# retab-dev/k-LLMs

Hardware: NVIDIA H100
Metric: consensus records/sec at n=16 (1M x 32-field); achieved HBM GB/s vs peak (higher is better)
Workload: dtype i32 codes / f64 values

## Files before the change

### k_llms_b200/csrc/kc_jsongpu.cu

```cuda
#include <cuda_runtime.h>

#include <algorithm>
#include <atomic>
#include <chrono>
#include <cstdio>
#include <cstdlib>
#include <cstring>
#include <mutex>
#include <string>
#include <thread>
#include <type_traits>
#include <vector>

#include <cub/device/device_scan.cuh>
#include <nvtx3/nvToolsExt.h>

#include "../../include/kllms_b200.h"
#include "kc_internal.h"
#include "kc_jsongpu.cuh"

namespace {

using kc::js::Chunk;
using kc::js::Tok;

#define R_(call)                              \
    do {                                      \
        if (const int rc_ = (call)) return rc_; \
    } while (0)

struct DBuf {
    void *p = nullptr;
    size_t cap = 0;
    int reserve(size_t need) {
        if (p && need <= cap) return KC_OK;
        if (p) cudaFree(p);
        p = nullptr;
        cap = 0;
        need += need / 8 + 256;
        if (cudaMalloc(&p, need) != cudaSuccess) {
            cudaGetLastError();
            return kc_fail(KC_ENOMEM, "kc_consolidate_json_packed: cudaMalloc(%zu) failed", need);
        }
        cap = need;
        return KC_OK;
    }
    int grow(size_t need, size_t keep, cudaStream_t s) {
        if (!keep) return reserve(need);
        if (p && need <= cap) return KC_OK;
        void *old = p;
        const size_t old_cap = cap;
        p = nullptr;
        cap = 0;
        if (const int rc = reserve(need)) {
            cudaFree(old);
            return rc;
        }
        if (old) KC_CUDA_I(cudaMemcpyAsync(p, old, std::min(keep, old_cap), cudaMemcpyDeviceToDevice, s));
        KC_CUDA_I(cudaStreamSynchronize(s));
        if (old) cudaFree(old);
        return KC_OK;
    }
    template <typename T>
    T *as() const { return static_cast<T *>(p); }
};

struct PBuf {
    void *p = nullptr;
    size_t cap = 0;
    int reserve(size_t need) {
        if (p && need <= cap) return KC_OK;
        if (p) cudaFreeHost(p);
        p = nullptr;
        cap = 0;
        need += need / 8 + 256;
        if (cudaHostAlloc(&p, need, cudaHostAllocDefault) != cudaSuccess) {
            cudaGetLastError();
            return kc_fail(KC_ENOMEM, "kc_consolidate_json_packed: cudaHostAlloc(%zu) failed", need);
        }
        cap = need;
        return KC_OK;
    }
    template <typename T>
    T *as() const { return static_cast<T *>(p); }
};

enum Stage { RECORDS, SLOTS, UNION, SCRATCH, CSR, OFF };
struct Units {
    size_t R, B, T = 0, P = 0, S = 0;
};
template <class Alloc>
int chunk_arrays(const Alloc &alloc, Chunk &ch, Stage stage, const Units &u, size_t keep, bool vrec) {
    const size_t n = (size_t)ch.n;
    int k = 0;
    auto a = [&](Stage st, auto *&ptr, size_t count, size_t per, size_t plus, int fill, bool on_device) {
        const int i = k++;
        return st == stage ? alloc(i, ptr, count * per + plus, keep * per, fill, on_device) : KC_OK;
    };
    R_(a(RECORDS, ch.fcount, u.R, 1, 1, 0, true));
    R_(a(RECORDS, ch.slot, u.R, 1, 1, 0, false));
    R_(a(RECORDS, ch.status, u.R, 1, 0, 0, false));
    R_(a(RECORDS, ch.nest, u.R, 1, 0, 0, false));
    R_(a(RECORDS, ch.pend, u.R, 1, 0, 0, false));
    R_(a(RECORDS, ch.plist, u.R, 1, 1, 0xFF, false));
    R_(a(ch.lists ? RECORDS : OFF, ch.lst, u.R, 1, 0, 0, false));
    R_(a(RECORDS, ch.vbase, u.R, 1, 0, 0, false));
    R_(a(RECORDS, ch.xbase, u.R, 1, 0, 0, false));
    R_(a(RECORDS, ch.mcount, u.R, 1, 1, 0, true));
    R_(a(RECORDS, ch.scount, u.R, 1, 1, 0, true));
    R_(a(RECORDS, ch.ccount, u.R, 1, 1, 0, true));
    R_(a(RECORDS, ch.len_c, u.R, 1, 1, 0, true));
    R_(a(RECORDS, ch.len_l, u.R, 1, 1, 0, true));
    R_(a(SLOTS, ch.toks, u.T, n, 1, 0, false));
    R_(a(SLOTS, ch.fdesc, u.T, 1, 1, 0, false));
    R_(a(SLOTS, ch.gpos, u.T, 1, 1, 0, false));
    R_(a(SLOTS, ch.piece_c, u.T, 1, 1, 0, false));
    R_(a(SLOTS, ch.piece_l, u.T, 1, 1, 0, false));
    R_(a(SLOTS, ch.vcells, u.T, n, 16, 0xFF, true));
    R_(a(SLOTS, ch.xcells, u.T, n, 2, 0, true));
    R_(a(vrec ? SLOTS : OFF, ch.vrec, u.T, 1, 1, 0xFF, false));
    R_(a(UNION, ch.ucand, u.P, n, 0, 0, false));
    R_(a(UNION, ch.ubase, u.P, 1, 0, 0, false));
    R_(a(UNION, ch.usize, u.P, 1, 0, 0, false));
    R_(a(SCRATCH, ch.utok, u.S, 1, 0, 0, false));
    R_(a(SCRATCH, ch.unode, u.S, 1, 0, 0, false));
    R_(a(SCRATCH, ch.umap, u.S, 1, 0, 0xFF, false));
    R_(a(CSR, ch.mchars, u.B, 1, 16, 0, false));
    R_(a(CSR, ch.mstr_off, u.T, n, 2, 0, false));
    R_(a(CSR, ch.mgrp_off, u.T, 1, 2, 0, false));
    return KC_OK;
}

void set_flags(Chunk &ch, uint32_t flags, uint8_t lists, int32_t aligned0) {
    ch.xmedoid = (flags & KC_JSON_NUMERIC_MEDOID) != 0;
    ch.key_union = (flags & KC_JSON_KEY_UNION) != 0;
    ch.unicode = (flags & KC_JSON_UNICODE) != 0;
    ch.lists = lists;
    ch.aligned0 = aligned0;
}

struct Worker {
    int device = -1;
    cudaStream_t stream = nullptr;
    cudaEvent_t ev[7] = {};
    DBuf text, off, counters, win, vmeta, xvalue, xmeta, out_c, out_l, scan_tmp, midx, mavg, seq, vweight;
    std::vector<DBuf> arrays;
    PBuf h_small;
    PBuf h_scan;
    bool busy = false;
    int init(int dev) {
        if (device == dev) return KC_OK;
        KC_CUDA_I(cudaStreamCreateWithFlags(&stream, cudaStreamNonBlocking));
        for (auto &e : ev) KC_CUDA_I(cudaEventCreate(&e));
        device = dev;
        return KC_OK;
    }
};

std::mutex g_pool_mu;
std::vector<Worker *> g_workers;

Worker *acquire_worker(int device) {
    std::lock_guard<std::mutex> lock(g_pool_mu);
    for (Worker *w : g_workers)
        if (!w->busy && w->device == device) {
            w->busy = true;
            return w;
        }
    Worker *w = new Worker;
    w->busy = true;
    g_workers.push_back(w);
    return w;
}
void release_worker(Worker *w) {
    std::lock_guard<std::mutex> lock(g_pool_mu);
    w->busy = false;
}

struct PinnedBlob {
    char *p = nullptr;
    size_t cap = 0;
};
std::vector<PinnedBlob> g_blob_pool;

PinnedBlob acquire_blob(size_t need) {
    {
        std::lock_guard<std::mutex> lock(g_pool_mu);
        int best = -1;
        for (int i = 0; i < (int)g_blob_pool.size(); ++i)
            if (g_blob_pool[i].cap >= need && (best < 0 || g_blob_pool[i].cap < g_blob_pool[best].cap)) best = i;
        if (best >= 0) {
            PinnedBlob b = g_blob_pool[best];
            g_blob_pool.erase(g_blob_pool.begin() + best);
            return b;
        }
    }
    PinnedBlob b;
    void *p = nullptr;
    if (cudaHostAlloc(&p, need, cudaHostAllocDefault) != cudaSuccess) {
        cudaGetLastError();
        return b;
    }
    b.p = (char *)p;
    b.cap = need;
    return b;
}
void release_blob(PinnedBlob b) {
    if (!b.p) return;
    std::lock_guard<std::mutex> lock(g_pool_mu);
    size_t n_small = 0, n_large = 0;
    for (auto &x : g_blob_pool) (x.cap <= ((size_t)4 << 20) ? n_small : n_large)++;
    if (b.cap <= ((size_t)4 << 20) && n_small < 64) {
        g_blob_pool.push_back(b);
        return;
    }
    if (n_large >= 4 || b.cap <= ((size_t)4 << 20)) {
        int smallest = -1;
        for (int i = 0; i < (int)g_blob_pool.size(); ++i)
            if (g_blob_pool[i].cap > ((size_t)4 << 20) && (smallest < 0 || g_blob_pool[i].cap < g_blob_pool[smallest].cap)) smallest = i;
        if (smallest < 0 || g_blob_pool[smallest].cap >= b.cap) {
            cudaFreeHost(b.p);
            return;
        }
        cudaFreeHost(g_blob_pool[smallest].p);
        g_blob_pool.erase(g_blob_pool.begin() + smallest);
    }
    g_blob_pool.push_back(b);
}

int team_size(int n) {
    int t = 2;
    while (t < n && t < 32) t *= 2;
    return t;
}

int device_arrays(Worker &w, Chunk &ch, Stage stage, const Units &u, size_t keep, bool weighted) {
    auto dev = [&](int k, auto *&ptr, size_t len, size_t keep_len, int fill, bool on_device) -> int {
        using E = std::remove_reference_t<decltype(*ptr)>;
        if (w.arrays.size() <= (size_t)k) w.arrays.resize((size_t)k + 1);
        R_(w.arrays[(size_t)k].grow(len * sizeof(E), keep_len * sizeof(E), w.stream));
        ptr = w.arrays[(size_t)k].as<E>();
        if (on_device) KC_CUDA_I(cudaMemsetAsync(ptr + keep_len, fill, (len - keep_len) * sizeof(E), w.stream));
        return KC_OK;
    };
    R_(chunk_arrays(dev, ch, stage, u, keep, weighted));
    if (stage != SLOTS) return KC_OK;
    const size_t T1 = std::max<size_t>(u.T, 1);
    R_(w.win.reserve(T1 * 4));
    R_(w.vmeta.reserve(T1 * 4));
    R_(w.xvalue.reserve(T1 * 8));
    R_(w.xmeta.reserve(T1 * 4));
    ch.vmeta = w.vmeta.as<uint32_t>();
    ch.xvalue = w.xvalue.as<double>();
    ch.xmeta = w.xmeta.as<uint32_t>();
    ch.xbest = w.xmeta.as<int32_t>();
    ch.xavg = w.xvalue.as<double>();
    if (weighted) {
        R_(w.vweight.reserve(T1 * 4));
        ch.vweight = w.vweight.as<float>();
    }
    return KC_OK;
}

template <typename T>
void exclusive_scan(T *v, size_t len) {
    T acc = 0;
    for (size_t i = 0; i < len; ++i) {
        const T c = v[i];
        v[i] = acc;
        acc += c;
    }
}

}

struct kc_json_result {
    int64_t R = 0;
    PinnedBlob blob;
    std::atomic<int64_t> used{0};
    std::vector<int64_t> c_off, c_len, l_off, l_len;
    std::vector<uint8_t> status, why;
    std::string heap;
    kc_json_stats stats{};
};

namespace {

struct ChunkStage {
    float h2d = 0, plan = 0, kernels = 0, emit = 0, d2h = 0;
};

int union_round(Worker &w, Chunk &ch, Units &u, int team, int grid, bool weighted, unsigned long long *h_cnt) {
    cudaStream_t s = w.stream;
    const int32_t P = (int32_t)u.P;
    R_(device_arrays(w, ch, UNION, u, 0, weighted));
    ch.uslot = (uint32_t)u.T;
    kc::js::union_count_kernel<<<grid, 128, 0, s>>>(ch, team, P);
    KC_CUDA_I(cudaGetLastError());
    KC_CUDA_I(cudaMemcpyAsync(h_cnt, ch.counters, 48, cudaMemcpyDeviceToHost, s));
    KC_CUDA_I(cudaStreamSynchronize(s));
    u.S = std::max<size_t>(h_cnt[4], 1);
    if (u.S >= ((size_t)1 << 32)) return kc_fail(KC_EINVAL, "kc_consolidate_json_packed: %zu union scratch entries in one chunk", u.S);
    R_(device_arrays(w, ch, SCRATCH, u, 0, weighted));
    kc::js::union_build_kernel<<<grid, 128, 0, s>>>(ch, team, P);
    KC_CUDA_I(cudaGetLastError());
    KC_CUDA_I(cudaMemcpyAsync(h_cnt, ch.counters, 48, cudaMemcpyDeviceToHost, s));
    KC_CUDA_I(cudaStreamSynchronize(s));
    if (const size_t U = h_cnt[5]) {
        const size_t keep = u.T;
        u.T += U;
        if (u.T >= ((size_t)1 << 32)) return kc_fail(KC_EINVAL, "kc_consolidate_json_packed: %zu field slots in one chunk", u.T);
        R_(device_arrays(w, ch, SLOTS, u, keep, weighted));
    }
    kc::js::union_plan_kernel<<<grid, 128, 0, s>>>(ch, team, P);
    KC_CUDA_I(cudaGetLastError());
    KC_CUDA_I(cudaMemcpyAsync(h_cnt, ch.counters, 48, cudaMemcpyDeviceToHost, s));
    KC_CUDA_I(cudaStreamSynchronize(s));
    return KC_OK;
}

int run_chunk(Worker &w, const char *h_text, const int64_t *h_off, const float *h_seq, uint32_t flags, uint8_t lists, const int64_t *dst,
              int64_t r0, int64_t r1, int32_t n, double rel_eps, double abs_eps, int sm_count, kc_json_result &res, ChunkStage &st) {
    const int64_t Rc = r1 - r0;
    const int64_t b0 = h_off[r0 * n], b1 = h_off[r1 * n];
    const size_t bytes = (size_t)(b1 - b0);
    if (bytes >= ((size_t)1 << 32)) return kc_fail(KC_EINVAL, "kc_consolidate_json_packed: chunk of %zu bytes", bytes);
    cudaStream_t s = w.stream;
    const bool weighted = h_seq != nullptr;
    Chunk ch{};
    ch.R = (int32_t)Rc;
    ch.n = n;
    set_flags(ch, flags, lists, INT32_MAX);
    Units u{(size_t)Rc, bytes};
    R_(device_arrays(w, ch, RECORDS, u, 0, weighted));
    R_(w.text.reserve(bytes + 16));
    R_(w.off.reserve((size_t)(Rc * n + 1) * 8));
    R_(w.counters.reserve(48));
    R_(w.h_small.reserve(64));
    R_(w.h_scan.reserve((size_t)(Rc + 1) * 16 + (size_t)Rc));
    if (h_seq) R_(w.seq.reserve((size_t)std::max<int64_t>(Rc * n, 1) * 4));
    size_t tmp_bytes = 0, tmp_bytes32 = 0;
    cub::DeviceScan::ExclusiveSum(nullptr, tmp_bytes, (const int64_t *)nullptr, (int64_t *)nullptr, (int)(Rc + 1), s);
    cub::DeviceScan::ExclusiveSum(nullptr, tmp_bytes32, (const uint32_t *)nullptr, (uint32_t *)nullptr, (int)(Rc + 1), s);
    R_(w.scan_tmp.reserve(std::max(tmp_bytes, tmp_bytes32) + 256));
    ch.text = w.text.as<uint8_t>();
    ch.off = w.off.as<int64_t>();
    ch.counters = w.counters.as<unsigned long long>();

    nvtxRangePushA("kc_json: H2D texts");
    KC_CUDA_I(cudaEventRecord(w.ev[0], s));
    KC_CUDA_I(cudaMemcpyAsync(w.text.p, h_text + b0, bytes, cudaMemcpyHostToDevice, s));
    KC_CUDA_I(cudaMemcpyAsync(w.off.p, h_off + r0 * n, (size_t)(Rc * n + 1) * 8, cudaMemcpyHostToDevice, s));
    if (h_seq) KC_CUDA_I(cudaMemcpyAsync(w.seq.p, h_seq + r0 * n, (size_t)(Rc * n) * 4, cudaMemcpyHostToDevice, s));
    KC_CUDA_I(cudaEventRecord(w.ev[1], s));
    nvtxRangePop();
    nvtxRangePushA("kc_json: plan (A0 count, A1 scan/type/encode)");

    const int team = team_size(n);
    const int tpw = 32 / team;
    auto grid_for = [&](int64_t threads_needed) {
        const int64_t blocks = (threads_needed + 127) / 128;
        return (int)std::max<int64_t>(1, std::min<int64_t>(blocks, (int64_t)sm_count * 16));
    };
    auto team_grid = [&](int64_t units) { return grid_for((units + tpw - 1) / tpw * 32); };
    kc::js::count_kernel<<<grid_for(Rc), 128, 0, s>>>(ch);
    KC_CUDA_I(cudaGetLastError());
    size_t tb = w.scan_tmp.cap;
    KC_CUDA_I(cub::DeviceScan::ExclusiveSum(w.scan_tmp.p, tb, (const uint32_t *)ch.fcount, ch.slot, (int)(Rc + 1), s));
    uint32_t *h_total = w.h_small.as<uint32_t>();
    KC_CUDA_I(cudaMemcpyAsync(h_total, ch.slot + Rc, 4, cudaMemcpyDeviceToHost, s));
    KC_CUDA_I(cudaStreamSynchronize(s));
    u.T = *h_total;
    R_(device_arrays(w, ch, SLOTS, u, 0, weighted));
    KC_CUDA_I(cudaMemsetAsync(w.counters.p, 0, 48, s));
    int64_t gv = 0, gx = 0, gm = 0;
    if (u.T) {
        kc::js::plan_kernel<<<team_grid(Rc), 128, 0, s>>>(ch, team);
        KC_CUDA_I(cudaGetLastError());
        unsigned long long *h_cnt = w.h_small.as<unsigned long long>() + 1;
        KC_CUDA_I(cudaMemcpyAsync(h_cnt, w.counters.p, 32, cudaMemcpyDeviceToHost, s));
        KC_CUDA_I(cudaStreamSynchronize(s));
        if ((u.P = h_cnt[3]))
            R_(union_round(w, ch, u, team, team_grid((int64_t)u.P), weighted, h_cnt));
        gv = (int64_t)h_cnt[0];
        gx = (int64_t)h_cnt[1];
        gm = (int64_t)h_cnt[2];
    }
    if (gm) {
        R_(device_arrays(w, ch, CSR, u, 0, weighted));
        R_(w.midx.reserve((u.T + 1) * 4));
        R_(w.mavg.reserve((u.T + 1) * 8));
        ch.midx = w.midx.as<int32_t>();
        ch.mavg = w.mavg.as<double>();
        for (uint32_t *cnt : {ch.mcount, ch.scount, ch.ccount}) {
            tb = w.scan_tmp.cap;
            KC_CUDA_I(cub::DeviceScan::ExclusiveSum(w.scan_tmp.p, tb, (const uint32_t *)cnt, cnt, (int)(Rc + 1), s));
        }
        kc::js::medoid_kernel<<<team_grid(Rc), 128, 0, s>>>(ch, team);
        KC_CUDA_I(cudaGetLastError());
    }
    KC_CUDA_I(cudaEventRecord(w.ev[2], s));
    nvtxRangePop();
    nvtxRangePushA("kc_json: K1 vote + K2 numeric + K4 medoid");
    if (gv && h_seq)
        R_(kc_weighted_vote_groups_i8(ch.vcells, gv, n, ch.vrec, w.seq.as<float>(), Rc, w.win.as<int32_t>(), w.vmeta.as<uint32_t>(),
                                      w.vweight.as<float>(), s));
    else if (gv)
        R_(kc_vote_i8(ch.vcells, gv, n, nullptr, 1, w.win.as<int32_t>(), w.vmeta.as<uint32_t>(), s));
    if (gx && ch.xmedoid) R_(kc_numeric_medoid_f64(ch.xcells, gx, n, w.xmeta.as<int32_t>(), w.xvalue.as<double>(), s));
    else if (gx) R_(kc_numeric_f64(ch.xcells, gx, n, rel_eps, abs_eps, w.xvalue.as<double>(), w.xmeta.as<uint32_t>(), s));
    if (gm) R_(kc_medoid_str(ch.mchars, ch.mstr_off, ch.mgrp_off, gm, std::max(2, n), w.midx.as<int32_t>(), w.mavg.as<double>(), s));
    KC_CUDA_I(cudaEventRecord(w.ev[3], s));
    nvtxRangePop();
    nvtxRangePushA("kc_json: emit (C0 lengths, C1 write)");
    kc::js::len_kernel<<<team_grid(Rc), 128, 0, s>>>(ch, team);
    KC_CUDA_I(cudaGetLastError());
    tb = w.scan_tmp.cap;
    KC_CUDA_I(cub::DeviceScan::ExclusiveSum(w.scan_tmp.p, tb, (const int64_t *)ch.len_c, ch.len_c, (int)(Rc + 1), s));
    tb = w.scan_tmp.cap;
    KC_CUDA_I(cub::DeviceScan::ExclusiveSum(w.scan_tmp.p, tb, (const int64_t *)ch.len_l, ch.len_l, (int)(Rc + 1), s));
    int64_t *h_scan_c = w.h_scan.as<int64_t>(), *h_scan_l = h_scan_c + (Rc + 1);
    uint8_t *h_status = (uint8_t *)(h_scan_l + (Rc + 1));
    KC_CUDA_I(cudaMemcpyAsync(h_scan_c, ch.len_c, (size_t)(Rc + 1) * 8, cudaMemcpyDeviceToHost, s));
    KC_CUDA_I(cudaMemcpyAsync(h_scan_l, ch.len_l, (size_t)(Rc + 1) * 8, cudaMemcpyDeviceToHost, s));
    KC_CUDA_I(cudaMemcpyAsync(h_status, ch.status, (size_t)Rc, cudaMemcpyDeviceToHost, s));
    KC_CUDA_I(cudaStreamSynchronize(s));
    const int64_t out_c_bytes = h_scan_c[Rc], out_l_bytes = h_scan_l[Rc];
    R_(w.out_c.reserve((size_t)std::max<int64_t>(out_c_bytes, 1)));
    R_(w.out_l.reserve((size_t)std::max<int64_t>(out_l_bytes, 1)));
    ch.out_c = w.out_c.as<uint8_t>();
    ch.out_l = w.out_l.as<uint8_t>();
    if (out_c_bytes) {
        kc::js::write_kernel<<<team_grid(Rc), 128, 0, s>>>(ch, team);
        KC_CUDA_I(cudaGetLastError());
    }
    KC_CUDA_I(cudaEventRecord(w.ev[4], s));
    nvtxRangePop();
    nvtxRangePushA("kc_json: D2H texts");
    const int64_t need = out_c_bytes + out_l_bytes;
    const int64_t pos = res.used.fetch_add(need);
    if (pos + need > (int64_t)res.blob.cap) {
        res.used.fetch_sub(need);
        for (int64_t i = r0; i < r1; ++i) {
            const int64_t r = dst ? dst[i] : i;
            res.status[(size_t)r] = 1;
            res.why[(size_t)r] = (uint8_t)kc::js::D_TOO_LONG;
        }
        return KC_OK;
    }
    if (out_c_bytes) KC_CUDA_I(cudaMemcpyAsync(res.blob.p + pos, ch.out_c, (size_t)out_c_bytes, cudaMemcpyDeviceToHost, s));
    if (out_l_bytes) KC_CUDA_I(cudaMemcpyAsync(res.blob.p + pos + out_c_bytes, ch.out_l, (size_t)out_l_bytes, cudaMemcpyDeviceToHost, s));
    KC_CUDA_I(cudaEventRecord(w.ev[5], s));
    KC_CUDA_I(cudaStreamSynchronize(s));
    nvtxRangePop();
    for (int64_t i = 0; i < Rc; ++i) {
        const int64_t r = dst ? dst[r0 + i] : r0 + i;
        res.status[(size_t)r] = h_status[i] ? 1 : 0;
        res.why[(size_t)r] = h_status[i];
        res.c_off[(size_t)r] = pos + h_scan_c[i];
        res.c_len[(size_t)r] = h_scan_c[i + 1] - h_scan_c[i];
        res.l_off[(size_t)r] = pos + out_c_bytes + h_scan_l[i];
        res.l_len[(size_t)r] = h_scan_l[i + 1] - h_scan_l[i];
    }
    float ms = 0;
    cudaEventElapsedTime(&ms, w.ev[0], w.ev[1]); st.h2d += ms;
    cudaEventElapsedTime(&ms, w.ev[1], w.ev[2]); st.plan += ms;
    cudaEventElapsedTime(&ms, w.ev[2], w.ev[3]); st.kernels += ms;
    cudaEventElapsedTime(&ms, w.ev[3], w.ev[4]); st.emit += ms;
    cudaEventElapsedTime(&ms, w.ev[4], w.ev[5]); st.d2h += ms;
    return KC_OK;
}

}

namespace {

void gather(const char *h_text, const int64_t *h_off, int32_t n, const std::vector<int64_t> &idx, std::vector<const char *> &texts,
            std::vector<int64_t> &lens) {
    texts.resize(idx.size() * n);
    lens.resize(idx.size() * n);
    for (size_t i = 0; i < idx.size(); ++i)
        for (int32_t c = 0; c < n; ++c) {
            const int64_t k = idx[i] * n + c;
            texts[i * n + c] = h_text + h_off[k];
            lens[i * n + c] = h_off[k + 1] - h_off[k];
        }
}

template <class Alloc>
int align_listed(const char *h_text, const int64_t *h_off, int32_t n, int device, int32_t threads, const std::vector<int64_t> &idx, const Alloc &alloc,
                 char *&blob, std::vector<int64_t> &off, std::vector<int64_t> &dst, std::vector<int64_t> &declined) {
    const int64_t L = (int64_t)idx.size();
    std::vector<const char *> texts;
    std::vector<int64_t> lens;
    gather(h_text, h_off, n, idx, texts, lens);
    std::vector<char *> out((size_t)(L * n), nullptr);
    std::vector<int32_t> st((size_t)L, 0);
    if (const int rc = kc_align_json_batch(texts.data(), lens.data(), L, n, 0.51, device, threads, out.data(), st.data(), nullptr)) {
        kc_free_strings(out.data(), L * n);
        return rc;
    }
    off.assign(1, 0);
    dst.clear();
    declined.clear();
    for (int64_t i = 0; i < L; ++i) {
        if (st[(size_t)i] != 0) {
            declined.push_back(idx[(size_t)i]);
            continue;
        }
        dst.push_back(idx[(size_t)i]);
        for (int32_t c = 0; c < n; ++c) off.push_back(off.back() + (int64_t)strlen(out[(size_t)(i * n + c)]));
    }
    blob = alloc((size_t)off.back());
    int rc = blob ? KC_OK : kc_fail(KC_ENOMEM, "kc_consolidate_json_packed: cannot allocate %lld bytes of aligned texts", (long long)off.back());
    for (int64_t i = 0, k = 0; i < L && !rc; ++i) {
        if (st[(size_t)i] != 0) continue;
        for (int32_t c = 0; c < n; ++c, ++k) memcpy(blob + off[(size_t)k], out[(size_t)(i * n + c)], (size_t)(off[(size_t)k + 1] - off[(size_t)k]));
    }
    kc_free_strings(out.data(), L * n);
    return rc;
}

template <class Round>
int list_round(kc_json_result &res, const char *h_text, const int64_t *h_off, const float *h_seq, int32_t n, int device, int32_t threads,
               Round &run_round) {
    std::vector<int64_t> idx;
    for (int64_t r = 0; r < res.R; ++r)
        if (res.status[(size_t)r] && res.why[(size_t)r] == kc::js::D_LIST) idx.push_back(r);
    if (idx.empty()) return KC_OK;
    PinnedBlob texts;
    auto alloc = [&](size_t bytes) {
        texts = acquire_blob(bytes + 16);
        return texts.p;
    };
    char *blob = nullptr;
    std::vector<int64_t> off, dst, declined;
    const int sim_device = idx.size() >= 64 ? device : -1;
    int rc = align_listed(h_text, h_off, n, sim_device, threads, idx, alloc, blob, off, dst, declined);
    for (int64_t r : declined) res.why[(size_t)r] = kc::js::D_ALIGN;
    const int64_t M = (int64_t)dst.size();
    if (!rc && M) {
        std::vector<float> seq;
        if (h_seq) {
            seq.resize((size_t)(M * n));
            for (int64_t i = 0; i < M; ++i) memcpy(&seq[(size_t)(i * n)], h_seq + dst[(size_t)i] * n, (size_t)n * 4);
        }
        size_t est = 4096;
        for (int64_t i = 0; i < M; ++i) {
            const char *t = blob + off[(size_t)(i * n)];
            const int64_t len = off[(size_t)(i * n + 1)] - off[(size_t)(i * n)];
            int64_t tokens = 1;
            for (int64_t k = 0; k < len; ++k) tokens += t[k] == ',' ? 1 : (t[k] == ']' || t[k] == '}') ? 2 : 0;
            est += (size_t)(2 * len + 32 * tokens);
        }
        const size_t need = (size_t)res.used.load() + est;
        if (need > res.blob.cap) {
            PinnedBlob bigger = acquire_blob(need);
            if (!bigger.p) rc = kc_fail(KC_ENOMEM, "kc_consolidate_json_packed: cannot grow the pinned output blob to %zu bytes", need);
            else {
                memcpy(bigger.p, res.blob.p, (size_t)res.used.load());
                release_blob(res.blob);
                res.blob = bigger;
            }
        }
        if (!rc) rc = run_round(blob, off.data(), h_seq ? seq.data() : nullptr, M, (uint8_t)2, dst.data());
    }
    release_blob(texts);
    return rc;
}

}

extern "C" {

namespace {

int consolidate_packed(const char *h_text, const int64_t *h_off, const float *h_seq, int64_t n_records, int32_t n, double rel_eps,
                       double abs_eps, int device, int32_t threads, uint32_t flags, kc_json_result **out) {
    if (!out) return kc_fail(KC_EINVAL, "kc_consolidate_json_packed: NULL out");
    if (h_seq || (flags & KC_JSON_NUMERIC_MEDOID)) flags |= KC_JSON_DEVICE_ONLY;
    *out = nullptr;
    if (n < 2 || n > KC_MAX_CANDIDATES) return kc_fail(KC_EINVAL, "kc_consolidate_json_packed: n=%d outside [2,%d]", n, KC_MAX_CANDIDATES);
    if (n_records < 0 || (n_records && (!h_text || !h_off))) return kc_fail(KC_EINVAL, "kc_consolidate_json_packed: bad arguments");
    if (!(rel_eps >= 0.0) || !(abs_eps >= 0.0)) return kc_fail(KC_EINVAL, "kc_consolidate_json_packed: rel_eps/abs_eps must be >= 0");
    const auto t_start = std::chrono::steady_clock::now();
    int prev = 0;
    KC_CUDA_I(cudaGetDevice(&prev));
    KC_CUDA_I(cudaSetDevice(device));
    int sm_count = 0, cc_major = 0;
    KC_CUDA_I(cudaDeviceGetAttribute(&sm_count, cudaDevAttrMultiProcessorCount, device));
    KC_CUDA_I(cudaDeviceGetAttribute(&cc_major, cudaDevAttrComputeCapabilityMajor, device));
    if (cc_major != 9) {
        cudaSetDevice(prev);
        return kc_fail(KC_ENODEV, "device %d has compute capability %d.x; this library is sm_90a only", device, cc_major);
    }
    kc_json_result *res = new (std::nothrow) kc_json_result;
    if (!res) return kc_fail(KC_ENOMEM, "kc_consolidate_json_packed: out of memory");
    const int64_t R = n_records;
    res->R = R;
    res->c_off.assign((size_t)R, 0);
    res->c_len.assign((size_t)R, 0);
    res->l_off.assign((size_t)R, 0);
    res->l_len.assign((size_t)R, 0);
    res->status.assign((size_t)R, 1);
    res->why.assign((size_t)R, 0);
    const int64_t total_bytes = R ? h_off[R * n] - h_off[0] : 0;
    res->blob = acquire_blob((size_t)(total_bytes / n * 3 + (1 << 20)));
    if (!res->blob.p) {
        delete res;
        cudaSetDevice(prev);
        return kc_fail(KC_ENOMEM, "kc_consolidate_json_packed: cannot allocate the pinned output blob");
    }
    size_t chunk_bytes = (size_t)64 << 20;
    if (const char *e = getenv("KC_JSON_CHUNK_MB")) chunk_bytes = (size_t)std::min(1024, std::max(1, atoi(e))) << 20;
    int max_workers = 3;
    if (const char *e = getenv("KC_JSON_STREAMS")) max_workers = std::max(1, std::min(8, atoi(e)));
    int n_chunks = 0, n_streams = 0;
    std::vector<ChunkStage> stages((size_t)max_workers);
    auto run_round = [&](const char *text, const int64_t *off, const float *seq, int64_t Rb, uint8_t lists, const int64_t *dst) -> int {
        std::vector<int64_t> cuts{0};
        int64_t r = 0;
        while (r < Rb) {
            const int64_t start = off[r * n];
            int64_t lo = r + 1, hi = Rb;
            while (lo < hi) {
                const int64_t mid = lo + (hi - lo + 1) / 2;
                if ((size_t)(off[mid * n] - start) <= chunk_bytes) lo = mid;
                else hi = mid - 1;
            }
            r = lo;
            cuts.push_back(r);
        }
        const int chunks = (int)cuts.size() - 1;
        const int n_workers = std::max(1, std::min(max_workers, chunks));
        n_chunks += chunks;
        n_streams = std::max(n_streams, n_workers);
        std::vector<Worker *> workers;
        for (int i = 0; i < n_workers; ++i) workers.push_back(acquire_worker(device));
        std::vector<int> rcs((size_t)n_workers, KC_OK);
        std::vector<std::string> errs((size_t)n_workers);
        std::atomic<int> next{0};
        auto body = [&](int wi) {
            cudaSetDevice(device);
            Worker &w = *workers[(size_t)wi];
            int rc = w.init(device);
            while (!rc) {
                const int k = next.fetch_add(1);
                if (k >= chunks) break;
                rc = run_chunk(w, text, off, seq, flags, lists, dst, cuts[(size_t)k], cuts[(size_t)k + 1], n, rel_eps, abs_eps, sm_count, *res,
                               stages[(size_t)wi]);
            }
            if (rc) {
                cudaStreamSynchronize(w.stream);
                errs[(size_t)wi] = kc_last_error();
            }
            rcs[(size_t)wi] = rc;
        };
        if (n_workers == 1) {
            body(0);
        } else {
            std::vector<std::thread> pool;
            for (int i = 0; i < n_workers; ++i) pool.emplace_back(body, i);
            for (auto &t : pool) t.join();
        }
        for (Worker *w : workers) release_worker(w);
        for (int i = 0; i < n_workers; ++i)
            if (rcs[(size_t)i]) return kc_fail(rcs[(size_t)i], "%s", errs[(size_t)i].c_str());
        return KC_OK;
    };
    const bool lists = (flags & KC_JSON_LISTS) != 0;
    int rc = run_round(h_text, h_off, h_seq, R, lists ? 1 : 0, nullptr);
    if (!rc && lists) rc = list_round(*res, h_text, h_off, h_seq, n, device, threads, run_round);
    const auto t_gpu = std::chrono::steady_clock::now();
    int64_t n_declined = 0, n_host = 0;
    if (!rc) {
        std::vector<int64_t> idx;
        for (int64_t r = 0; r < R; ++r) {
            if (!res->status[(size_t)r]) continue;
            ++n_declined;
            if (res->why[(size_t)r] != kc::js::D_ALIGN) idx.push_back(r);
        }
        if (!idx.empty() && !(flags & KC_JSON_DEVICE_ONLY)) {
            const int64_t D = (int64_t)idx.size();
            std::vector<const char *> texts;
            std::vector<int64_t> lens;
            gather(h_text, h_off, n, idx, texts, lens);
            std::vector<char *> oc((size_t)D, nullptr), ol((size_t)D, nullptr);
            std::vector<uint8_t> hs((size_t)D, 1);
            rc = kc_consolidate_json(texts.data(), lens.data(), D, n, rel_eps, abs_eps, device, threads, oc.data(), ol.data(), hs.data());
            if (!rc) {
                int64_t pos = res->used.load(), extra = 0;
                for (int64_t i = 0; i < D; ++i)
                    if (hs[(size_t)i] == 0) extra += (int64_t)(strlen(oc[(size_t)i]) + strlen(ol[(size_t)i]));
                char *base = res->blob.p;
                if (pos + extra > (int64_t)res->blob.cap) {
                    res->heap.resize((size_t)(pos + extra));
                    memcpy(&res->heap[0], res->blob.p, (size_t)pos);
                    release_blob(res->blob);
                    res->blob = PinnedBlob{};
                    base = &res->heap[0];
                }
                for (int64_t i = 0; i < D; ++i) {
                    if (hs[(size_t)i] != 0) continue;
                    const int64_t r = idx[(size_t)i];
                    const size_t lc = strlen(oc[(size_t)i]), ll = strlen(ol[(size_t)i]);
                    memcpy(base + pos, oc[(size_t)i], lc);
                    memcpy(base + pos + lc, ol[(size_t)i], ll);
                    res->c_off[(size_t)r] = pos;
                    res->l_off[(size_t)r] = pos + (int64_t)lc;
                    res->c_len[(size_t)r] = (int64_t)lc;
                    res->l_len[(size_t)r] = (int64_t)ll;
                    res->status[(size_t)r] = 2;
                    pos += (int64_t)(lc + ll);
                    ++n_host;
                }
                res->used.store(pos);
            }
            kc_free_strings(oc.data(), D);
            kc_free_strings(ol.data(), D);
        }
    }
    cudaSetDevice(prev);
    if (rc) {
        release_blob(res->blob);
        delete res;
        return rc;
    }
    const auto t_end = std::chrono::steady_clock::now();
    auto ms = [](auto a, auto b) { return std::chrono::duration<double, std::milli>(b - a).count(); };
    kc_json_stats &s = res->stats;
    s.n_records = R;
    s.n_device = R - n_declined;
    s.n_host = n_host;
    s.n_python = n_declined - n_host;
    s.input_bytes = total_bytes;
    s.output_bytes = res->used.load();
    s.chunks = n_chunks;
    s.streams = n_streams;
    for (auto &g : stages) {
        s.h2d_ms += g.h2d;
        s.plan_ms += g.plan;
        s.kernel_ms += g.kernels;
        s.emit_ms += g.emit;
        s.d2h_ms += g.d2h;
    }
    s.device_path_wall_ms = ms(t_start, t_gpu);
    s.host_path_wall_ms = ms(t_gpu, t_end);
    s.wall_ms = ms(t_start, t_end);
    *out = res;
    return KC_OK;
}

}

int kc_consolidate_json_packed(const char *h_text, const int64_t *h_off, int64_t n_records, int32_t n, double rel_eps, double abs_eps,
                               int device, int32_t threads, uint32_t flags, kc_json_result **out) {
    return consolidate_packed(h_text, h_off, nullptr, n_records, n, rel_eps, abs_eps, device, threads, flags, out);
}

int kc_consolidate_json_packed_weighted(const char *h_text, const int64_t *h_off, const float *h_seq_logprob, int64_t n_records, int32_t n,
                                        double rel_eps, double abs_eps, int device, int32_t threads, uint32_t flags, kc_json_result **out) {
    if (n_records > 0 && !h_seq_logprob) return kc_fail(KC_EINVAL, "kc_consolidate_json_packed_weighted: NULL h_seq_logprob");
    static const float none = 0.0f;
    return consolidate_packed(h_text, h_off, h_seq_logprob ? h_seq_logprob : &none, n_records, n, rel_eps, abs_eps, device, threads, flags, out);
}

int kc_json_result_view(kc_json_result *res, const char **text, const int64_t **content_off, const int64_t **content_len,
                        const int64_t **likelihoods_off, const int64_t **likelihoods_len, const uint8_t **status, const uint8_t **why,
                        kc_json_stats *stats) {
    if (!res) return kc_fail(KC_EINVAL, "kc_json_result_view: NULL result");
    if (text) *text = res->blob.p ? res->blob.p : res->heap.data();
    if (content_off) *content_off = res->c_off.data();
    if (content_len) *content_len = res->c_len.data();
    if (likelihoods_off) *likelihoods_off = res->l_off.data();
    if (likelihoods_len) *likelihoods_len = res->l_len.data();
    if (status) *status = res->status.data();
    if (why) *why = res->why.data();
    if (stats) *stats = res->stats;
    return KC_OK;
}

void kc_json_result_free(kc_json_result *res) {
    if (!res) return;
    release_blob(res->blob);
    delete res;
}


struct kc_debug_jsongpu {
    std::vector<int64_t> off;
    std::vector<uint8_t> text;
    int32_t n = 0;
    int64_t R = 0;
    std::vector<std::vector<uint8_t>> arrays;
    unsigned long long counters[6] = {0, 0, 0, 0, 0, 0};
    std::vector<uint8_t> out_c, out_l;
    int64_t R_out = 0;
    std::vector<int64_t> src;
    std::vector<int64_t> spliced_c, spliced_l;
    std::vector<uint8_t> spliced_out_c, spliced_out_l;
    Chunk ch{};
};

int kc_debug_jsongpu_plan(const char *h_text, const int64_t *h_off, int64_t n_records, int32_t n, kc_debug_jsongpu **out) {
    return kc_debug_jsongpu_plan_flags(h_text, h_off, n_records, n, 0u, out);
}

namespace {

void plan_twin(kc_debug_jsongpu *h, const char *h_text, const int64_t *h_off, int64_t R, int32_t n, uint32_t flags, uint8_t lists, int32_t aligned0) {
    h->R = R;
    h->R_out = R;
    h->n = n;
    h->off.assign(h_off, h_off + R * n + 1);
    h->text.assign((const uint8_t *)h_text + h_off[0], (const uint8_t *)h_text + h_off[R * n]);
    Chunk &ch = h->ch;
    ch.text = h->text.data();
    ch.off = h->off.data();
    ch.R = (int32_t)R;
    ch.n = n;
    ch.counters = h->counters;
    set_flags(ch, flags, lists, aligned0);
    auto host = [&](int k, auto *&ptr, size_t len, size_t, int fill, bool) -> int {
        using E = std::remove_reference_t<decltype(*ptr)>;
        if (h->arrays.size() <= (size_t)k) h->arrays.resize((size_t)k + 1);
        h->arrays[(size_t)k].resize(len * sizeof(E), (uint8_t)fill);
        ptr = reinterpret_cast<E *>(h->arrays[(size_t)k].data());
        return KC_OK;
    };
    Units u{(size_t)R, h->text.size()};
    chunk_arrays(host, ch, RECORDS, u, 0, true);
    for (int32_t r = 0; r < R; ++r) kc::js::count_record(ch, r);
    for (int64_t r = 0; r < R; ++r) ch.slot[r + 1] = ch.slot[r] + ch.fcount[r];
    u.T = ch.slot[R];
    chunk_arrays(host, ch, SLOTS, u, 0, true);
    const kc::js::HostTeam team{team_size(n)};
    for (int32_t r = 0; r < R; ++r) kc::js::plan_step(ch, r, team);
    if ((u.P = h->counters[3])) {
        const int32_t P = (int32_t)u.P;
        chunk_arrays(host, ch, UNION, u, 0, true);
        ch.uslot = (uint32_t)u.T;
        for (int32_t p = 0; p < P; ++p) kc::js::union_count_step(ch, p, team);
        u.S = std::max<size_t>(h->counters[4], 1);
        chunk_arrays(host, ch, SCRATCH, u, 0, true);
        for (int32_t p = 0; p < P; ++p) kc::js::union_build_step(ch, p, team);
        const size_t keep = u.T;
        u.T += h->counters[5];
        chunk_arrays(host, ch, SLOTS, u, keep, true);
        for (int32_t p = 0; p < P; ++p) kc::js::union_plan_step(ch, p, team);
    }
    for (uint32_t *cnt : {ch.mcount, ch.scount, ch.ccount}) exclusive_scan(cnt, u.R + 1);
    chunk_arrays(host, ch, CSR, u, 0, true);
    for (int32_t r = 0; r < R; ++r) kc::js::medoid_step(ch, r, team);
}

}

int kc_debug_jsongpu_plan_flags(const char *h_text, const int64_t *h_off, int64_t n_records, int32_t n, uint32_t flags,
                                kc_debug_jsongpu **out) {
    if (!h_text || !h_off || !out || n < 2 || n > KC_MAX_CANDIDATES || n_records < 0) return KC_EINVAL;
    const int64_t R = n_records;
    kc_debug_jsongpu *h = new kc_debug_jsongpu;
    const bool lists = (flags & KC_JSON_LISTS) != 0;
    plan_twin(h, h_text, h_off, R, n, flags, lists ? 1 : 0, INT32_MAX);
    std::vector<int64_t> idx;
    for (int64_t r = 0; r < R && lists; ++r)
        if (h->ch.status[r] == kc::js::D_LIST) idx.push_back(r);
    if (idx.empty()) {
        *out = h;
        return KC_OK;
    }
    std::vector<char> aligned;
    auto alloc = [&](size_t bytes) {
        aligned.resize(bytes + 1);
        return aligned.data();
    };
    char *blob = nullptr;
    std::vector<int64_t> aoff, dst, declined;
    if (const int rc = align_listed(h_text, h_off, n, -1, 0, idx, alloc, blob, aoff, dst, declined)) {
        delete h;
        return rc;
    }
    const int64_t M = (int64_t)dst.size(), base = h_off[R * n] - h_off[0];
    std::vector<char> text(h_text + h_off[0], h_text + h_off[R * n]);
    text.insert(text.end(), blob, blob + aoff.back());
    std::vector<int64_t> off((size_t)((R + M) * n + 1));
    for (int64_t k = 0; k <= R * n; ++k) off[(size_t)k] = h_off[k] - h_off[0];
    for (int64_t k = 1; k <= M * n; ++k) off[(size_t)(R * n + k)] = base + aoff[(size_t)k];
    delete h;
    h = new kc_debug_jsongpu;
    plan_twin(h, text.data(), off.data(), R + M, n, flags, 1, (int32_t)R);
    h->R_out = R;
    h->src = dst;
    for (int64_t r : declined) h->ch.status[r] = kc::js::D_ALIGN;
    int32_t *vrec = h->ch.vrec;
    for (uint64_t g = 0; g < h->counters[0]; ++g)
        if (vrec[g] >= R) vrec[g] = (int32_t)dst[(size_t)(vrec[g] - R)];
    *out = h;
    return KC_OK;
}

int kc_debug_jsongpu_medoid_inputs(const kc_debug_jsongpu *h, const uint8_t **chars, const int32_t **str_off, const int32_t **grp_off,
                                   int64_t *n_groups) {
    if (!h) return KC_EINVAL;
    if (chars) *chars = h->ch.mchars;
    if (str_off) *str_off = h->ch.mstr_off;
    if (grp_off) *grp_off = h->ch.mgrp_off;
    if (n_groups) *n_groups = (int64_t)h->counters[2];
    return KC_OK;
}

int kc_debug_jsongpu_set_medoid(kc_debug_jsongpu *h, const int32_t *medoid_idx, const double *medoid_avg) {
    if (!h) return KC_EINVAL;
    h->ch.midx = medoid_idx;
    h->ch.mavg = medoid_avg;
    return KC_OK;
}

int kc_debug_jsongpu_set_numeric_medoid(kc_debug_jsongpu *h, const int32_t *best, const double *best_avg) {
    if (!h) return KC_EINVAL;
    h->ch.xbest = best;
    h->ch.xavg = best_avg;
    return KC_OK;
}

int kc_debug_jsongpu_inputs(const kc_debug_jsongpu *h, const int8_t **vote_cells, int64_t *n_vote_groups, const double **num_cells,
                            int64_t *n_num_groups, const uint8_t **status) {
    if (!h) return KC_EINVAL;
// ... 298 lines not shown
```

Before: 1.020 billion.

## Double-buffer chunk uploads on a separate copy stream to overlap with compute

Each worker now holds two sets of device buffers for text, offsets and sequence weights plus a pinned staging buffer. While the current chunk runs on the compute stream, the next chunk's inputs are uploaded on a dedicated copy stream, synchronised with events. Offsets and weights are first copied into pinned staging memory so those transfers can be truly asynchronous. This aims to hide H2D transfer time behind compute, at the cost of doubled input buffers and extra host memcpy work.

```diff
diff --git a/k_llms_b200/csrc/kc_jsongpu.cu b/k_llms_b200/csrc/kc_jsongpu.cu
--- a/k_llms_b200/csrc/kc_jsongpu.cu
+++ b/k_llms_b200/csrc/kc_jsongpu.cu
@@ -141,9 +141,12 @@
 
 struct Worker {
     int device = -1;
-    cudaStream_t stream = nullptr;
+    cudaStream_t stream = nullptr, copy = nullptr;
     cudaEvent_t ev[7] = {};
-    DBuf text, off, counters, win, vmeta, xvalue, xmeta, out_c, out_l, scan_tmp, midx, mavg, seq, vweight;
+    cudaEvent_t copy_start[2] = {}, copied[2] = {}, enqueued = nullptr;
+    DBuf text[2], off[2], seq[2];
+    PBuf stage[2];
+    DBuf counters, win, vmeta, xvalue, xmeta, out_c, out_l, scan_tmp, midx, mavg, vweight;
     std::vector<DBuf> arrays;
     PBuf h_small;
     PBuf h_scan;
@@ -151,7 +154,13 @@
     int init(int dev) {
         if (device == dev) return KC_OK;
         KC_CUDA_I(cudaStreamCreateWithFlags(&stream, cudaStreamNonBlocking));
+        KC_CUDA_I(cudaStreamCreateWithFlags(&copy, cudaStreamNonBlocking));
         for (auto &e : ev) KC_CUDA_I(cudaEventCreate(&e));
+        for (int b = 0; b < 2; ++b) {
+            KC_CUDA_I(cudaEventCreate(&copy_start[b]));
+            KC_CUDA_I(cudaEventCreate(&copied[b]));
+        }
+        KC_CUDA_I(cudaEventCreateWithFlags(&enqueued, cudaEventDisableTiming));
         device = dev;
         return KC_OK;
     }
@@ -319,41 +328,53 @@
     return KC_OK;
 }
 
-int run_chunk(Worker &w, const char *h_text, const int64_t *h_off, const float *h_seq, uint32_t flags, uint8_t lists, const int64_t *dst,
+int prefetch(Worker &w, int b, const char *h_text, const int64_t *h_off, const float *h_seq, int64_t r0, int64_t r1, int32_t n) {
+    const int64_t Rc = r1 - r0;
+    const int64_t b0 = h_off[r0 * n];
+    const size_t bytes = (size_t)(h_off[r1 * n] - b0);
+    if (bytes >= ((size_t)1 << 32)) return kc_fail(KC_EINVAL, "kc_consolidate_json_packed: chunk of %zu bytes", bytes);
+    const size_t off_bytes = (size_t)(Rc * n + 1) * 8, seq_bytes = h_seq ? (size_t)(Rc * n) * 4 : 0;
+    R_(w.text[b].reserve(bytes + 16));
+    R_(w.off[b].reserve(off_bytes));
+    R_(w.stage[b].reserve(off_bytes + seq_bytes));
+    if (h_seq) R_(w.seq[b].reserve(std::max<size_t>(seq_bytes, 4)));
+    int64_t *h_off_st = w.stage[b].as<int64_t>();
+    memcpy(h_off_st, h_off + r0 * n, off_bytes);
+    if (h_seq) memcpy(h_off_st + Rc * n + 1, h_seq + r0 * n, seq_bytes);
+    KC_CUDA_I(cudaEventRecord(w.enqueued, w.stream));
+    KC_CUDA_I(cudaStreamWaitEvent(w.copy, w.enqueued, 0));
+    KC_CUDA_I(cudaEventRecord(w.copy_start[b], w.copy));
+    KC_CUDA_I(cudaMemcpyAsync(w.text[b].p, h_text + b0, bytes, cudaMemcpyHostToDevice, w.copy));
+    KC_CUDA_I(cudaMemcpyAsync(w.off[b].p, h_off_st, off_bytes, cudaMemcpyHostToDevice, w.copy));
+    if (h_seq) KC_CUDA_I(cudaMemcpyAsync(w.seq[b].p, h_off_st + Rc * n + 1, seq_bytes, cudaMemcpyHostToDevice, w.copy));
+    KC_CUDA_I(cudaEventRecord(w.copied[b], w.copy));
+    return KC_OK;
+}
+
+int run_chunk(Worker &w, int b, const int64_t *h_off, bool weighted, uint32_t flags, uint8_t lists, const int64_t *dst,
               int64_t r0, int64_t r1, int32_t n, double rel_eps, double abs_eps, int sm_count, kc_json_result &res, ChunkStage &st) {
     const int64_t Rc = r1 - r0;
-    const int64_t b0 = h_off[r0 * n], b1 = h_off[r1 * n];
-    const size_t bytes = (size_t)(b1 - b0);
-    if (bytes >= ((size_t)1 << 32)) return kc_fail(KC_EINVAL, "kc_consolidate_json_packed: chunk of %zu bytes", bytes);
+    const size_t bytes = (size_t)(h_off[r1 * n] - h_off[r0 * n]);
     cudaStream_t s = w.stream;
-    const bool weighted = h_seq != nullptr;
     Chunk ch{};
     ch.R = (int32_t)Rc;
     ch.n = n;
     set_flags(ch, flags, lists, INT32_MAX);
     Units u{(size_t)Rc, bytes};
     R_(device_arrays(w, ch, RECORDS, u, 0, weighted));
-    R_(w.text.reserve(bytes + 16));
-    R_(w.off.reserve((size_t)(Rc * n + 1) * 8));
     R_(w.counters.reserve(48));
     R_(w.h_small.reserve(64));
     R_(w.h_scan.reserve((size_t)(Rc + 1) * 16 + (size_t)Rc));
-    if (h_seq) R_(w.seq.reserve((size_t)std::max<int64_t>(Rc * n, 1) * 4));
     size_t tmp_bytes = 0, tmp_bytes32 = 0;
     cub::DeviceScan::ExclusiveSum(nullptr, tmp_bytes, (const int64_t *)nullptr, (int64_t *)nullptr, (int)(Rc + 1), s);
     cub::DeviceScan::ExclusiveSum(nullptr, tmp_bytes32, (const uint32_t *)nullptr, (uint32_t *)nullptr, (int)(Rc + 1), s);
     R_(w.scan_tmp.reserve(std::max(tmp_bytes, tmp_bytes32) + 256));
-    ch.text = w.text.as<uint8_t>();
-    ch.off = w.off.as<int64_t>();
+    ch.text = w.text[b].as<uint8_t>();
+    ch.off = w.off[b].as<int64_t>();
     ch.counters = w.counters.as<unsigned long long>();
 
-    nvtxRangePushA("kc_json: H2D texts");
-    KC_CUDA_I(cudaEventRecord(w.ev[0], s));
-    KC_CUDA_I(cudaMemcpyAsync(w.text.p, h_text + b0, bytes, cudaMemcpyHostToDevice, s));
-    KC_CUDA_I(cudaMemcpyAsync(w.off.p, h_off + r0 * n, (size_t)(Rc * n + 1) * 8, cudaMemcpyHostToDevice, s));
-    if (h_seq) KC_CUDA_I(cudaMemcpyAsync(w.seq.p, h_seq + r0 * n, (size_t)(Rc * n) * 4, cudaMemcpyHostToDevice, s));
+    KC_CUDA_I(cudaStreamWaitEvent(s, w.copied[b], 0));
     KC_CUDA_I(cudaEventRecord(w.ev[1], s));
-    nvtxRangePop();
     nvtxRangePushA("kc_json: plan (A0 count, A1 scan/type/encode)");
 
     const int team = team_size(n);
@@ -402,8 +423,8 @@
     KC_CUDA_I(cudaEventRecord(w.ev[2], s));
     nvtxRangePop();
     nvtxRangePushA("kc_json: K1 vote + K2 numeric + K4 medoid");
-    if (gv && h_seq)
-        R_(kc_weighted_vote_groups_i8(ch.vcells, gv, n, ch.vrec, w.seq.as<float>(), Rc, w.win.as<int32_t>(), w.vmeta.as<uint32_t>(),
+    if (gv && weighted)
+        R_(kc_weighted_vote_groups_i8(ch.vcells, gv, n, ch.vrec, w.seq[b].as<float>(), Rc, w.win.as<int32_t>(), w.vmeta.as<uint32_t>(),
                                       w.vweight.as<float>(), s));
     else if (gv)
         R_(kc_vote_i8(ch.vcells, gv, n, nullptr, 1, w.win.as<int32_t>(), w.vmeta.as<uint32_t>(), s));
@@ -463,7 +484,7 @@
         res.l_len[(size_t)r] = h_scan_l[i + 1] - h_scan_l[i];
     }
     float ms = 0;
-    cudaEventElapsedTime(&ms, w.ev[0], w.ev[1]); st.h2d += ms;
+    cudaEventElapsedTime(&ms, w.copy_start[b], w.copied[b]); st.h2d += ms;
     cudaEventElapsedTime(&ms, w.ev[1], w.ev[2]); st.plan += ms;
     cudaEventElapsedTime(&ms, w.ev[2], w.ev[3]); st.kernels += ms;
     cudaEventElapsedTime(&ms, w.ev[3], w.ev[4]); st.emit += ms;
@@ -644,13 +665,19 @@
             cudaSetDevice(device);
             Worker &w = *workers[(size_t)wi];
             int rc = w.init(device);
-            while (!rc) {
-                const int k = next.fetch_add(1);
-                if (k >= chunks) break;
-                rc = run_chunk(w, text, off, seq, flags, lists, dst, cuts[(size_t)k], cuts[(size_t)k + 1], n, rel_eps, abs_eps, sm_count, *res,
-                               stages[(size_t)wi]);
+            int k = rc ? chunks : next.fetch_add(1), b = 0;
+            if (k < chunks) rc = prefetch(w, b, text, off, seq, cuts[(size_t)k], cuts[(size_t)k + 1], n);
+            while (!rc && k < chunks) {
+                const int k_next = next.fetch_add(1);
+                if (k_next < chunks) rc = prefetch(w, b ^ 1, text, off, seq, cuts[(size_t)k_next], cuts[(size_t)k_next + 1], n);
+                if (!rc)
+                    rc = run_chunk(w, b, off, seq != nullptr, flags, lists, dst, cuts[(size_t)k], cuts[(size_t)k + 1], n, rel_eps, abs_eps, sm_count,
+                                   *res, stages[(size_t)wi]);
+                k = k_next;
+                b ^= 1;
             }
             if (rc) {
+                cudaStreamSynchronize(w.copy);
                 cudaStreamSynchronize(w.stream);
                 errs[(size_t)wi] = kc_last_error();
             }
```

Result: no change. 1.022 billion, median of 6 (+0.1%).

## Double-buffer chunk uploads on a separate copy stream to overlap H2D with compute

Applied to the files above, without the earlier changes.

Adds two upload slots per worker and a dedicated copy stream, so the next chunk's text, offsets and sequence logprobs upload while the current chunk's kernels run. Events order slot reuse between the two streams. Offsets are staged through a pinned host buffer so that copy can run asynchronously. It also stops zero-initialising the per-record output arrays by using uninitialised unique_ptr arrays, with an explicit zeroing added on the too-long path. The cost is doubled device upload buffers plus extra event synchronisation, and other paths that relied on the old zeroing may now leave garbage.

```diff
diff --git a/k_llms_b200/csrc/kc_jsongpu.cu b/k_llms_b200/csrc/kc_jsongpu.cu
--- a/k_llms_b200/csrc/kc_jsongpu.cu
+++ b/k_llms_b200/csrc/kc_jsongpu.cu
@@ -6,6 +6,7 @@
 #include <cstdio>
 #include <cstdlib>
 #include <cstring>
+#include <memory>
 #include <mutex>
 #include <string>
 #include <thread>
@@ -139,11 +140,19 @@
     ch.aligned0 = aligned0;
 }
 
+struct Slot {
+    DBuf text, off, seq;
+    PBuf h_off;
+    cudaEvent_t start = nullptr, filled = nullptr, released = nullptr;
+};
+
 struct Worker {
     int device = -1;
     cudaStream_t stream = nullptr;
+    cudaStream_t copy = nullptr;
     cudaEvent_t ev[7] = {};
-    DBuf text, off, counters, win, vmeta, xvalue, xmeta, out_c, out_l, scan_tmp, midx, mavg, seq, vweight;
+    Slot slot[2];
+    DBuf counters, win, vmeta, xvalue, xmeta, out_c, out_l, scan_tmp, midx, mavg, vweight;
     std::vector<DBuf> arrays;
     PBuf h_small;
     PBuf h_scan;
@@ -151,9 +160,29 @@
     int init(int dev) {
         if (device == dev) return KC_OK;
         KC_CUDA_I(cudaStreamCreateWithFlags(&stream, cudaStreamNonBlocking));
+        KC_CUDA_I(cudaStreamCreateWithFlags(&copy, cudaStreamNonBlocking));
         for (auto &e : ev) KC_CUDA_I(cudaEventCreate(&e));
+        for (Slot &sl : slot) {
+            KC_CUDA_I(cudaEventCreate(&sl.start));
+            KC_CUDA_I(cudaEventCreate(&sl.filled));
+            KC_CUDA_I(cudaEventCreateWithFlags(&sl.released, cudaEventDisableTiming));
+        }
         device = dev;
         return KC_OK;
+    }
+    int size_slots(size_t bytes, int64_t Rc, int32_t n, bool weighted) {
+        if (bytes >= ((size_t)1 << 32)) return kc_fail(KC_EINVAL, "kc_consolidate_json_packed: chunk of %zu bytes", bytes);
+        for (Slot &sl : slot) {
+            R_(sl.text.reserve(bytes + 16));
+            R_(sl.off.reserve((size_t)(Rc * n + 1) * 8));
+            R_(sl.h_off.reserve((size_t)(Rc * n + 1) * 8));
+            if (weighted) R_(sl.seq.reserve((size_t)std::max<int64_t>(Rc * n, 1) * 4));
+        }
+        return KC_OK;
+    }
+    void drain() {
+        cudaStreamSynchronize(copy);
+        cudaStreamSynchronize(stream);
     }
 };
 
@@ -278,7 +307,7 @@
     int64_t R = 0;
     PinnedBlob blob;
     std::atomic<int64_t> used{0};
-    std::vector<int64_t> c_off, c_len, l_off, l_len;
+    std::unique_ptr<int64_t[]> c_off, c_len, l_off, l_len;
     std::vector<uint8_t> status, why;
     std::string heap;
     kc_json_stats stats{};
@@ -319,12 +348,27 @@
     return KC_OK;
 }
 
-int run_chunk(Worker &w, const char *h_text, const int64_t *h_off, const float *h_seq, uint32_t flags, uint8_t lists, const int64_t *dst,
+int upload(Worker &w, Slot &sl, const char *h_text, const int64_t *h_off, const float *h_seq, int32_t n, int64_t r0, int64_t r1) {
+    const int64_t Rc = r1 - r0;
+    const int64_t b0 = h_off[r0 * n], b1 = h_off[r1 * n];
+    const size_t off_bytes = (size_t)(Rc * n + 1) * 8;
+    nvtxRangePushA("kc_json: H2D texts");
+    KC_CUDA_I(cudaEventSynchronize(sl.filled));
+    memcpy(sl.h_off.p, h_off + r0 * n, off_bytes);
+    KC_CUDA_I(cudaStreamWaitEvent(w.copy, sl.released, 0));
+    KC_CUDA_I(cudaEventRecord(sl.start, w.copy));
+    KC_CUDA_I(cudaMemcpyAsync(sl.text.p, h_text + b0, (size_t)(b1 - b0), cudaMemcpyHostToDevice, w.copy));
+    KC_CUDA_I(cudaMemcpyAsync(sl.off.p, sl.h_off.p, off_bytes, cudaMemcpyHostToDevice, w.copy));
+    if (h_seq) KC_CUDA_I(cudaMemcpyAsync(sl.seq.p, h_seq + r0 * n, (size_t)(Rc * n) * 4, cudaMemcpyHostToDevice, w.copy));
+    KC_CUDA_I(cudaEventRecord(sl.filled, w.copy));
+    nvtxRangePop();
+    return KC_OK;
+}
+
+int run_chunk(Worker &w, Slot &sl, const int64_t *h_off, const float *h_seq, uint32_t flags, uint8_t lists, const int64_t *dst,
               int64_t r0, int64_t r1, int32_t n, double rel_eps, double abs_eps, int sm_count, kc_json_result &res, ChunkStage &st) {
     const int64_t Rc = r1 - r0;
-    const int64_t b0 = h_off[r0 * n], b1 = h_off[r1 * n];
-    const size_t bytes = (size_t)(b1 - b0);
-    if (bytes >= ((size_t)1 << 32)) return kc_fail(KC_EINVAL, "kc_consolidate_json_packed: chunk of %zu bytes", bytes);
+    const size_t bytes = (size_t)(h_off[r1 * n] - h_off[r0 * n]);
     cudaStream_t s = w.stream;
     const bool weighted = h_seq != nullptr;
     Chunk ch{};
@@ -333,27 +377,19 @@
     set_flags(ch, flags, lists, INT32_MAX);
     Units u{(size_t)Rc, bytes};
     R_(device_arrays(w, ch, RECORDS, u, 0, weighted));
-    R_(w.text.reserve(bytes + 16));
-    R_(w.off.reserve((size_t)(Rc * n + 1) * 8));
     R_(w.counters.reserve(48));
     R_(w.h_small.reserve(64));
     R_(w.h_scan.reserve((size_t)(Rc + 1) * 16 + (size_t)Rc));
-    if (h_seq) R_(w.seq.reserve((size_t)std::max<int64_t>(Rc * n, 1) * 4));
     size_t tmp_bytes = 0, tmp_bytes32 = 0;
     cub::DeviceScan::ExclusiveSum(nullptr, tmp_bytes, (const int64_t *)nullptr, (int64_t *)nullptr, (int)(Rc + 1), s);
     cub::DeviceScan::ExclusiveSum(nullptr, tmp_bytes32, (const uint32_t *)nullptr, (uint32_t *)nullptr, (int)(Rc + 1), s);
     R_(w.scan_tmp.reserve(std::max(tmp_bytes, tmp_bytes32) + 256));
-    ch.text = w.text.as<uint8_t>();
-    ch.off = w.off.as<int64_t>();
+    ch.text = sl.text.as<uint8_t>();
+    ch.off = sl.off.as<int64_t>();
     ch.counters = w.counters.as<unsigned long long>();
 
-    nvtxRangePushA("kc_json: H2D texts");
-    KC_CUDA_I(cudaEventRecord(w.ev[0], s));
-    KC_CUDA_I(cudaMemcpyAsync(w.text.p, h_text + b0, bytes, cudaMemcpyHostToDevice, s));
-    KC_CUDA_I(cudaMemcpyAsync(w.off.p, h_off + r0 * n, (size_t)(Rc * n + 1) * 8, cudaMemcpyHostToDevice, s));
-    if (h_seq) KC_CUDA_I(cudaMemcpyAsync(w.seq.p, h_seq + r0 * n, (size_t)(Rc * n) * 4, cudaMemcpyHostToDevice, s));
+    KC_CUDA_I(cudaStreamWaitEvent(s, sl.filled, 0));
     KC_CUDA_I(cudaEventRecord(w.ev[1], s));
-    nvtxRangePop();
     nvtxRangePushA("kc_json: plan (A0 count, A1 scan/type/encode)");
 
     const int team = team_size(n);
@@ -403,7 +439,7 @@
     nvtxRangePop();
     nvtxRangePushA("kc_json: K1 vote + K2 numeric + K4 medoid");
     if (gv && h_seq)
-        R_(kc_weighted_vote_groups_i8(ch.vcells, gv, n, ch.vrec, w.seq.as<float>(), Rc, w.win.as<int32_t>(), w.vmeta.as<uint32_t>(),
+        R_(kc_weighted_vote_groups_i8(ch.vcells, gv, n, ch.vrec, sl.seq.as<float>(), Rc, w.win.as<int32_t>(), w.vmeta.as<uint32_t>(),
                                       w.vweight.as<float>(), s));
     else if (gv)
         R_(kc_vote_i8(ch.vcells, gv, n, nullptr, 1, w.win.as<int32_t>(), w.vmeta.as<uint32_t>(), s));
@@ -445,6 +481,7 @@
             const int64_t r = dst ? dst[i] : i;
             res.status[(size_t)r] = 1;
             res.why[(size_t)r] = (uint8_t)kc::js::D_TOO_LONG;
+            if (!dst) res.c_off[(size_t)r] = res.c_len[(size_t)r] = res.l_off[(size_t)r] = res.l_len[(size_t)r] = 0;
         }
         return KC_OK;
     }
@@ -463,7 +500,7 @@
         res.l_len[(size_t)r] = h_scan_l[i + 1] - h_scan_l[i];
     }
     float ms = 0;
-    cudaEventElapsedTime(&ms, w.ev[0], w.ev[1]); st.h2d += ms;
+    cudaEventElapsedTime(&ms, sl.start, sl.filled); st.h2d += ms;
     cudaEventElapsedTime(&ms, w.ev[1], w.ev[2]); st.plan += ms;
     cudaEventElapsedTime(&ms, w.ev[2], w.ev[3]); st.kernels += ms;
     cudaEventElapsedTime(&ms, w.ev[3], w.ev[4]); st.emit += ms;
@@ -598,10 +635,7 @@
     if (!res) return kc_fail(KC_ENOMEM, "kc_consolidate_json_packed: out of memory");
     const int64_t R = n_records;
     res->R = R;
-    res->c_off.assign((size_t)R, 0);
-    res->c_len.assign((size_t)R, 0);
-    res->l_off.assign((size_t)R, 0);
-    res->l_len.assign((size_t)R, 0);
+    for (auto *v : {&res->c_off, &res->c_len, &res->l_off, &res->l_len}) v->reset(new int64_t[(size_t)R]);
     res->status.assign((size_t)R, 1);
     res->why.assign((size_t)R, 0);
     const int64_t total_bytes = R ? h_off[R * n] - h_off[0] : 0;
@@ -635,6 +669,12 @@
         const int n_workers = std::max(1, std::min(max_workers, chunks));
         n_chunks += chunks;
         n_streams = std::max(n_streams, n_workers);
+        size_t max_bytes = 0;
+        int64_t max_records = 0;
+        for (int k = 0; k < chunks; ++k) {
+            max_bytes = std::max(max_bytes, (size_t)(off[cuts[(size_t)k + 1] * n] - off[cuts[(size_t)k] * n]));
+            max_records = std::max(max_records, cuts[(size_t)k + 1] - cuts[(size_t)k]);
+        }
         std::vector<Worker *> workers;
         for (int i = 0; i < n_workers; ++i) workers.push_back(acquire_worker(device));
         std::vector<int> rcs((size_t)n_workers, KC_OK);
@@ -644,16 +684,21 @@
             cudaSetDevice(device);
             Worker &w = *workers[(size_t)wi];
             int rc = w.init(device);
-            while (!rc) {
-                const int k = next.fetch_add(1);
-                if (k >= chunks) break;
-                rc = run_chunk(w, text, off, seq, flags, lists, dst, cuts[(size_t)k], cuts[(size_t)k + 1], n, rel_eps, abs_eps, sm_count, *res,
-                               stages[(size_t)wi]);
+            if (!rc) rc = w.size_slots(max_bytes, max_records, n, seq != nullptr);
+            int k = next.fetch_add(1), cur = 0;
+            if (!rc && k < chunks) rc = upload(w, w.slot[cur], text, off, seq, n, cuts[(size_t)k], cuts[(size_t)k + 1]);
+            while (!rc && k < chunks) {
+                const int k_next = next.fetch_add(1);
+                if (k_next < chunks) rc = upload(w, w.slot[cur ^ 1], text, off, seq, n, cuts[(size_t)k_next], cuts[(size_t)k_next + 1]);
+                if (!rc)
+                    rc = run_chunk(w, w.slot[cur], off, seq, flags, lists, dst, cuts[(size_t)k], cuts[(size_t)k + 1], n, rel_eps, abs_eps, sm_count,
+                                   *res, stages[(size_t)wi]);
+                cudaEventRecord(w.slot[cur].released, w.stream);
+                k = k_next;
+                cur ^= 1;
             }
-            if (rc) {
-                cudaStreamSynchronize(w.stream);
-                errs[(size_t)wi] = kc_last_error();
-            }
+            w.drain();
+            if (rc) errs[(size_t)wi] = kc_last_error();
             rcs[(size_t)wi] = rc;
         };
         if (n_workers == 1) {
@@ -770,10 +815,10 @@
                         kc_json_stats *stats) {
     if (!res) return kc_fail(KC_EINVAL, "kc_json_result_view: NULL result");
     if (text) *text = res->blob.p ? res->blob.p : res->heap.data();
-    if (content_off) *content_off = res->c_off.data();
-    if (content_len) *content_len = res->c_len.data();
-    if (likelihoods_off) *likelihoods_off = res->l_off.data();
-    if (likelihoods_len) *likelihoods_len = res->l_len.data();
+    if (content_off) *content_off = res->c_off.get();
+    if (content_len) *content_len = res->c_len.get();
+    if (likelihoods_off) *likelihoods_off = res->l_off.get();
+    if (likelihoods_len) *likelihoods_len = res->l_len.get();
     if (status) *status = res->status.data();
     if (why) *why = res->why.data();
     if (stats) *stats = res->stats;
```

Measured after the change: 1.025 billion before, 1.025 billion after (median of 6 runs). No clear change (+0.0%).
